# axruff/cuda-flow3d

Hardware: AMD Instinct MI355X
Metric: Mvoxels/s full pyramid solve (higher is better)
Workload: dtype f32; 1 GPU; 512^3 synthetic translated-Gaussian float32 pair (BASELINE config 4), full coarse-to-fine pyramid (40 levels x 40 outer x 5 inner, alpha 7.5, median 5^3, Gaussian sigma 2), frames resident in HBM (value = device-resident rate); parallelism=1 GPU

## Files before the change

cuda-flow3d_amd/__init__.py:

```python
import atexit
import collections
import contextlib
import ctypes as C
import os
import weakref

import numpy as np

_HERE = os.path.dirname(os.path.abspath(__file__))
_LIBDIR = os.environ.get("F3D_LIBDIR") or os.path.join(_HERE, "lib")

DEFAULT_PARAMS = dict(
    warp_levels_count=40, warp_scale_factor=0.95, outer_iterations_count=40, inner_iterations_count=5,
    equation_alpha=7.5, equation_smoothness=0.001, equation_data=0.001, median_radius=5, gaussian_sigma=2.0,
)


class F3dError(RuntimeError):
    pass


class Size4(C.Structure):
    _fields_ = [("width", C.c_size_t), ("height", C.c_size_t), ("depth", C.c_size_t), ("pitch", C.c_size_t)]

# ... 265 lines not shown
        "f3d_flow_principal_compute": [C.c_void_p, C.c_int, C.c_uint, C.POINTER(_fp), C.POINTER(PrincipalStats)],
        "f3d_flow_principal_end": [C.c_void_p],
        "f3d_flow_polar_compute": [C.c_void_p, C.c_int, C.c_uint, C.POINTER(_fp), C.POINTER(PolarStats)],
        "f3d_flow_polar_end": [C.c_void_p],
        "f3d_flow_inverse_compute": [C.c_void_p, C.c_int, C.c_uint, C.c_float, C.POINTER(_fp), C.POINTER(InverseStats)],
        "f3d_flow_inverse_end": [C.c_void_p],
        "f3d_flow_match_compute": [C.c_void_p, C.c_int, C.c_uint, C.c_uint, C.c_float, C.POINTER(_fp), C.POINTER(CorrelationStats)],
        "f3d_flow_match_end": [C.c_void_p],
        "f3d_motion_solve": [C.POINTER(MotionSums), C.c_int, C.POINTER(MotionFit)],
        "f3d_motion_solve_labels": [C.POINTER(MotionSums), _sz, C.c_int, C.c_ulonglong, C.POINTER(C.c_double), C.POINTER(MotionFit),
                                    C.POINTER(C.c_int)],
        "f3d_flow_motion_compute": [C.c_void_p, C.c_int, C.c_int, C.c_float, C.POINTER(_fp), C.POINTER(MotionFit),
                                    C.POINTER(MotionResidual)],
        "f3d_flow_motion_end": [C.c_void_p],
        "f3d_flow_label_motion_compute": [C.c_void_p, C.c_int, C.POINTER(C.c_int), _sz, C.c_int, C.c_ulonglong, C.POINTER(_fp),
                                          C.POINTER(MotionFit), C.POINTER(C.c_int), C.POINTER(C.c_double), C.POINTER(LabelInfo)],
        "f3d_flow_label_motion_end": [C.c_void_p],
        "f3d_flow_validate_compute": [C.c_void_p, C.c_int, C.c_uint, C.c_float, C.c_float, C.c_uint, C.c_uint, C.c_uint, C.c_float,
                                      C.POINTER(_fp), C.POINTER(ValidateStats)],
        "f3d_flow_validate_end": [C.c_void_p],
        "f3d_op_create": [C.POINTER(C.c_void_p), C.c_char_p], "f3d_op_initialize": [C.c_void_p, C.POINTER(Size4)],
        "f3d_op_execute": [C.c_void_p, C.POINTER(C.c_char_p), C.POINTER(C.c_void_p), _sz],
        "f3d_op_execute_batch": [C.c_void_p, C.POINTER(C.c_char_p), C.POINTER(C.c_void_p), C.POINTER(_sz), _sz],
        "f3d_op_set_slab": [C.c_void_p, _slabp], "f3d_op_destroy": [C.c_void_p],
        "f3d_level_geometry": [_sz, _sz, _sz, C.c_float, C.c_int, C.POINTER(Size4), _fp, _fp, _fp],
        "f3d_gaussian_taps": [C.c_float, _fp, _sz, C.POINTER(_sz)],
        "f3d_raw_read_u8": [C.c_char_p, _sz, _sz, _sz, _fp], "f3d_raw_read_f32": [C.c_char_p, _sz, _sz, _sz, _fp],
        "f3d_raw_write_u8": [C.c_char_p, _fp, _sz, _sz, _sz], "f3d_raw_write_f32": [C.c_char_p, _fp, _sz, _sz, _sz],
        "f3d_vtk_write_flow": [C.c_char_p, _fp, _fp, _fp, _sz, _sz, _sz],
        "f3d_synth_pair": [_sz, _sz, _sz, _fp, _fp],
        "f3d_synth_planes": [_sz, _sz, _sz, _sz, _sz, _fp, _fp, _fp],
        "f3d_slabflow_create": [C.POINTER(C.c_void_p), C.c_int, C.POINTER(C.c_int), C.c_int, C.c_int],
        "f3d_slabflow_initialize": [C.c_void_p, _sz, _sz, _sz],
        "f3d_slabflow_compute": [C.c_void_p, _fp, _fp, pp, _fp, _fp, _fp],
        "f3d_slabflow_upload": [C.c_void_p, _fp, _fp],
        "f3d_slabflow_compute_resident": [C.c_void_p, pp, _fp],
        "f3d_slabflow_download": [C.c_void_p, _fp, _fp, _fp],
        "f3d_slabflow_overlapped_iterations": [C.c_void_p, C.POINTER(_sz)],
        "f3d_slabflow_batched_exchanges": [C.c_void_p, C.POINTER(_sz)],
        "f3d_slabflow_gathered_warps": [C.c_void_p, C.POINTER(_sz)],
        "f3d_slabflow_stage_exchanges": [C.c_void_p, C.POINTER(_sz)],
        "f3d_slabflow_set_exchange_per_stage": [C.c_void_p, C.c_int],
        "f3d_slabflow_destroy": [C.c_void_p],
        "f3d_plan_owned": [C.c_int, C.c_int, C.c_int, C.POINTER(C.c_int), C.POINTER(C.c_int)],
        "f3d_plan_exchange": [C.c_int] * 5 + [C.POINTER(C.c_int)] * 5 + [C.c_int],
        "f3d_plan_resample_source": [C.c_int] * 4 + [C.POINTER(C.c_int)] * 2,
        "f3d_volume_wrap": [C.POINTER(C.c_void_p), _fp, _sz, _sz, _sz], "f3d_volume_destroy": [C.c_void_p],
        "f3d_op_solve_p_last": [C.c_void_p, C.POINTER(C.c_int), C.POINTER(C.c_int), C.POINTER(C.c_int), C.POINTER(_sz), C.POINTER(C.c_int)],
        "f3d_op_solve_p_fused_weights": [C.c_void_p, C.POINTER(C.c_int)],
        "f3d_plan_solve_piecemeal": [_sz, _sz, _sz, C.c_int, C.c_int, C.c_int, C.c_int, C.c_int] + [C.POINTER(C.c_int)] * 5,
        "f3d_plan_sweeps": [C.c_int] * 4 + [C.POINTER(C.c_int)] * 2 + [C.c_int],
        "f3d_pair8_plan": [C.c_int] * 7 + [C.POINTER(C.c_longlong)],
        "f3d_pair8_decode": [C.c_int] * 4 + [C.POINTER(C.c_longlong)] + [C.c_int] * 5 + [C.POINTER(C.c_int)] * 2,
        "f3d_pflow_create": [C.POINTER(C.c_void_p)], "f3d_pflow_initialize": [C.c_void_p, _sz, _sz, _sz],
        "f3d_pflow_compute": [C.c_void_p, _fp, _fp, _sz, _sz, _sz, pp, C.c_int, _fp, _fp, _fp, _fp],
        "f3d_pflow_stats": [C.c_void_p, C.POINTER(_sz), C.POINTER(_sz), C.POINTER(_sz)], "f3d_pflow_destroy": [C.c_void_p],
        "f3d_pflow_set_resident": [C.c_void_p, C.c_int], "f3d_pflow_set_full_pipeline": [C.c_void_p, C.c_int], "f3d_pflow_originals_on_device": [C.c_void_p, C.POINTER(C.c_int)],
        "f3d_pflow_operator_seconds": [C.c_void_p, C.POINTER(C.c_double)],
        "f3d_pflow_levels_registered_inside": [C.c_void_p, C.POINTER(_sz)],
        "f3d_pflow_levels_with_constants_on_device": [C.c_void_p, C.POINTER(_sz)],
        "f3d_host_shutdown": [],
    }
    for name, args in sig.items():
        try:
            fn = getattr(L, name)
        except AttributeError:
            if os.environ.get("F3D_LIBDIR"):
                continue
            raise
        fn.argtypes = args
        fn.restype = C.c_int
    L.f3d_flow_default_params.argtypes = [pp]
    L.f3d_flow_default_params.restype = None
    L.f3d_op_name.argtypes = [C.c_void_p]
    L.f3d_op_name.restype = C.c_char_p
    L.f3d_max_warp_level.argtypes = [_sz, _sz, _sz, C.c_float]
    L.f3d_max_warp_level.restype = _sz
    L.f3d_volume_object.argtypes = [C.c_void_p]
    L.f3d_volume_object.restype = C.c_void_p
    L.f3d_volume_data.argtypes = [C.c_void_p]
    L.f3d_volume_data.restype = C.c_void_p
    L.f3d_piecemeal_budget_bytes.argtypes = []
    L.f3d_piecemeal_budget_bytes.restype = _sz
    if hasattr(L, "f3d_host_last_error"):
        L.f3d_host_last_error.argtypes = []
        L.f3d_host_last_error.restype = C.c_char_p
    _host = L
    return L


def shutdown():
    HostVolume.release_all()
    if _host is not None:
        _host.f3d_host_shutdown()
    elif _hip is not None and _hip.f3d_is_initialized():
        _hip.f3d_comm_destroy()
        _hip.f3d_shutdown()


atexit.register(shutdown)


def check(status, what="f3d call"):
    if status != 0:
        msg = hip().f3d_last_error()
        raise F3dError(f"{what} failed: {msg.decode() if msg else 'status %d' % status}")
# ... 688 lines not shown
    @property
    def object(self):
        return host().f3d_volume_object(self._h)

    @property
    def array(self):
        return HostVolume._storage[host().f3d_volume_data(self._h)][0]

    def destroy(self):
        if self._h:
            fin = getattr(self, "_finalizer", None)
            if fin is not None:
                fin.detach()
            HostVolume._release(self._h.value)
            self._h = C.c_void_p()


def plan_solve_piecemeal(budget_bytes, width, height, depth, inner_iterations, outer_iterations, forced_outer_per_pass=0,
                         overlap_mode=0):
    out = [C.c_int() for _ in range(5)]
    check(host().f3d_plan_solve_piecemeal(budget_bytes, width, height, depth, inner_iterations, outer_iterations,
                                          forced_outer_per_pass, overlap_mode, *[C.byref(o) for o in out]))
    return tuple(o.value for o in out)


def plan_sweeps(inner, fused, tri, carry):
    cap = max(1, inner)
    sweeps, weights = (C.c_int * cap)(), (C.c_int * cap)()
    n = host().f3d_plan_sweeps(inner, int(bool(fused)), int(bool(tri)), int(bool(carry)), sweeps, weights, cap)
    if n < 0:
        raise F3dError("f3d_plan_sweeps failed")
    return [(sweeps[i], bool(weights[i])) for i in range(n)]


Pair8Plan = collections.namedtuple("Pair8Plan", "A a b zc_a zc_b wgs cost tiles")


def pair8_plan(width, rows, planes, ty, zc_limit=None, per_round=0, fold=False):
    out = (C.c_longlong * 8)()
    check(host().f3d_pair8_plan(width, rows, planes, ty, planes if zc_limit is None else zc_limit, per_round, int(bool(fold)), out))
    return Pair8Plan(*[int(v) for v in out])


def pair8_decode(width, rows, ty, fold, plan, xcd_remap, z_lo, z_hi):
    cut = (C.c_longlong * 8)(*plan)
    grid = C.c_int()
    args = (width, rows, ty, int(bool(fold)), cut, int(bool(xcd_remap)), z_lo, z_hi)
    check(host().f3d_pair8_decode(*args, 0, 0, None, C.byref(grid)))
    out = np.empty((grid.value, 6), np.int32)
    check(host().f3d_pair8_decode(*args, 0, grid.value, out.ctypes.data_as(C.POINTER(C.c_int)), None))
    return out


class Operation:

    def __init__(self, name):
        self._h = C.c_void_p()
        if host().f3d_op_create(C.byref(self._h), name.encode()) != 0:
            raise F3dError(f"unknown operation {name!r}")
        self.values = {}

    @property
    def name(self):
        return host().f3d_op_name(self._h).decode()

    def initialize(self, containers=None):
        if containers is None:
            return host().f3d_op_initialize(self._h, None) == 0
        s = containers.size4
        return host().f3d_op_initialize(self._h, C.byref(s)) == 0

    def set_slab(self, slab):
        self._slab = slab
        host().f3d_op_set_slab(self._h, C.byref(slab) if slab is not None else None)

    def execute(self, **params):
        store = {}
        volumes = {}
        for k, v in params.items():
            if isinstance(v, HostVolume):
                volumes[k] = v
            elif k in _PTR_KEYS:
                store[k] = _dp(v)
            elif k in _SIZE_T_KEYS:
                store[k] = _sz(v)
            elif k in _FLOAT_KEYS:
                store[k] = C.c_float(v)
            elif k in _SIZE4_KEYS:
                store[k] = Size4(v[0], v[1], v[2], 0) if not isinstance(v, Size4) else v
            elif k == "max_mag":
                store[k] = _sz(v)
            elif k == "stat":
                store[k] = v
            elif k == "flow_update":
                store[k] = C.c_bool(bool(v))
            else:
                raise TypeError(f"unknown parameter key {k!r}")
        n = len(store) + len(volumes)
        keys = (C.c_char_p * n)(*[k.encode() for k in list(store) + list(volumes)])
        ptrs = (C.c_void_p * n)(*([C.cast(C.byref(v), C.c_void_p) for v in store.values()] +
                                  [C.c_void_p(v.object) for v in volumes.values()]))
        check(host().f3d_op_execute(self._h, keys, ptrs, n), "f3d_op_execute")
        self.values = {k: (v.value if hasattr(v, "value") else v) for k, v in store.items()}
        return self.values

    def execute_batch(self, bags):
# ... 463 lines not shown
```

cuda-flow3d_amd/csrc/f3d_pair8_plan.h:

```cpp
#pragma once

#include <algorithm>
#include <cstdlib>

#if !defined(__HIPCC__) && !defined(__host__)
#define __host__
#define __device__
#define F3D_PAIR8_PLAN_OWN_QUALIFIERS
#endif

constexpr int kPair8Lanes = 64;

__host__ __device__ inline int pair8_tiles_per_chunk(int ntx, int nty, bool fold)
{
  return fold ? (ntx - 1) * nty + (nty + 1) / 2 : ntx * nty;
}
inline bool pair8_folds(int width, int rows, int ty)
{
  const char* e = std::getenv("F3D_PAIR8_FOLD");
  if (e && e[0] == '0') return false;
  const int rem = width % kPair8Lanes;
  return rem >= 1 && rem <= kPair8Lanes / 2 && width > kPair8Lanes && rows > ty;
}

struct Pair8Cut {
  int tiles_a, chunks_a, zc_a;
  int tiles_b, chunks_b, zc_b;
};
__host__ __device__ inline int pair8_cut_wgs(const Pair8Cut& c) { return c.tiles_a * c.chunks_a + c.tiles_b * c.chunks_b; }
__host__ __device__ inline int pair8_cut_grid(const Pair8Cut& c, int xcd_remap)
{
  if (!xcd_remap) return pair8_cut_wgs(c);
  return 8 * ((c.tiles_a * c.chunks_a + 7) / 8 + (c.tiles_b * c.chunks_b + 7) / 8);
}

struct Pair8Wg {
  int tile;
  int tx, ty;
  bool folded;
  int z0, z1;
};

__host__ __device__ inline bool pair8_decode(int wg, const Pair8Cut& c, int ntx, int nty, bool fold, int xcd_remap, int m_lo,
                                             int m_hi, int more, Pair8Wg& w)
{
  const int n_a = c.tiles_a * c.chunks_a, n_b = c.tiles_b * c.chunks_b;
  bool in_a;
  int item;
  if (xcd_remap) {
    const int per_a = (n_a + 7) / 8, per_b = (n_b + 7) / 8;
    const int xcd = wg % 8, s = wg / 8;
    in_a = s < per_a;
    item = in_a ? xcd * per_a + s : xcd * per_b + (s - per_a);
  } else {
    in_a = wg < n_a;
    item = in_a ? wg : wg - n_a;
  }
  if (item >= (in_a ? n_a : n_b)) return false;
  const int tiles = in_a ? c.tiles_a : c.tiles_b, zc = in_a ? c.zc_a : c.zc_b;
  const int chunk = item / tiles;
  w.tile = item % tiles + (in_a ? 0 : c.tiles_a);
  w.z0 = m_lo + chunk * zc;
  w.z1 = w.z0 + zc + more < m_hi ? w.z0 + zc + more : m_hi;
  if (fold) {
    const int pair = w.tile / (2 * ntx - 1), k = w.tile % (2 * ntx - 1);
    w.folded = k == ntx - 1;
    w.tx = k < ntx ? k : k - ntx;
    w.ty = k < ntx ? 2 * pair : 2 * pair + 1;
  } else {
    w.folded = false;
    w.tx = w.tile % ntx;
    w.ty = w.tile / ntx;
  }
  return true;
}

struct Pair8Plan {
  int zchunk;
  long cost;
  long wgs = 0;
  Pair8Cut cut = {};
};
inline Pair8Cut pair8_uniform_cut(int tiles, int planes, int zchunk)
{
  return Pair8Cut{0, 0, 0, tiles, (planes + zchunk - 1) / zchunk, zchunk};
}
inline long pair8_per_round(long standard)
{
  const char* e = std::getenv("F3D_PAIR8_ROUND");
  const long v = e ? std::atol(e) : 0;
  return v > 0 ? v : standard;
}
inline Pair8Plan pair8_plan_dims(int width, int rows, int planes, int ty, int zc_limit, long per_round = 256, bool fold = false,
                                 bool two_class = true)
{
  const long tiles = pair8_tiles_per_chunk((width + kPair8Lanes - 1) / kPair8Lanes, (rows + ty - 1) / ty, fold);
  const int max_chunks = planes > 0 ? planes : 1;
  static const int extra = std::getenv("F3D_PAIR8_CHUNK_STEPS") ? std::atoi(std::getenv("F3D_PAIR8_CHUNK_STEPS")) : 7;
  auto rounds = [&](long wgs) { return (wgs + per_round - 1) / per_round; };
  Pair8Plan p = {std::min(planes, zc_limit), -1};
  for (int nzc = 1; nzc <= max_chunks; ++nzc) {
    const int zc = (planes + nzc - 1) / nzc;
    if (zc > zc_limit) continue;
    const long wgs = tiles * ((planes + zc - 1) / zc);
    const long cost = rounds(wgs) * (zc + extra);
    if (p.cost < 0 || cost < p.cost) {
      p.cost = cost;
      p.zchunk = zc;
      p.wgs = wgs;
    }
  }
  if (p.cost < 0) {
    p.cost = static_cast<long>(rounds(tiles)) * (p.zchunk + extra);
    p.wgs = tiles;
  }
  if (p.zchunk < 1) p.zchunk = 1;
  p.cut = pair8_uniform_cut(static_cast<int>(tiles), planes, p.zchunk);
  const char* pe = std::getenv("F3D_PAIR8_PLAN");
  if (!two_class || (pe && pe[0] == '0') || tiles <= per_round || planes < 1 || zc_limit < 1) return p;
  const int a0 = (planes + zc_limit - 1) / zc_limit;
  int zc_a_seen = 0;
  for (int na = a0; na <= a0 + 2 && na <= planes; ++na) {
    const int zc_a = (planes + na - 1) / na;
    if (zc_a > zc_limit || zc_a == zc_a_seen) continue;
    zc_a_seen = zc_a;
    const int a = (planes + zc_a - 1) / zc_a;
    long g = a, r = per_round;
    while (r) { const long t = g % r; g = r; r = t; }
    const long stride = per_round / g;
    for (long A = stride; A < tiles; A += stride) {
      const long cost_a = rounds(A * a) * (zc_a + extra);
      if (cost_a >= p.cost) break;
      int zc_b_seen = 0;
      for (int nb = 1; nb <= planes; ++nb) {
        const int zc_b = (planes + nb - 1) / nb;
        if (zc_b > zc_limit || zc_b == zc_b_seen) continue;
        zc_b_seen = zc_b;
        const int b = (planes + zc_b - 1) / zc_b;
        const long cost = cost_a + rounds((tiles - A) * b) * (zc_b + extra);
        if (cost < p.cost) {
          p.cost = cost;
          p.wgs = A * a + (tiles - A) * b;
          p.cut = Pair8Cut{static_cast<int>(A), a, zc_a, static_cast<int>(tiles - A), b, zc_b};
        }
      }
    }
  }
  return p;
}

#ifdef F3D_PAIR8_PLAN_OWN_QUALIFIERS
#undef __host__
#undef __device__
#undef F3D_PAIR8_PLAN_OWN_QUALIFIERS
#endif
```

cuda-flow3d_amd/csrc/f3d_solve_pair8.h:

```cpp

enum { PAIR_SS = 0, PAIR_SP = 1 };

struct PairArgs {
  const float* in[12];
  float* out[5];
  float hx, hy, hz, alpha;
  float eps_s, eps_d;
  int plain_division;
  int keep_below, keep_above;
  double r4[3], r2[3];
  float d4[3], d2[3];
  float w[3];
  float eps_s2, eps_d2;
  int fdivs_ok, sdivs_ok;
};

inline bool pair_weights_finite(float hx, float hy, float hz, float alpha)
{
  for (float h : {hx, hy, hz}) {
    const float w = alpha / (h * h);
    if (!(w - w == 0.f) || std::signbit(w)) return false;
  }
  return true;
}
// ... 656 lines not shown
    fetch_neighbours(colw_c, Sp);
  };

  __syncthreads();
  PlaneRegs A = {}, B = {}, Cc = {};
  const float* Sm = &ring[0][0];
  const float* S0 = &ring[1][0];
  using Slot0 = std::integral_constant<int, 0>;
  using Slot1 = std::integral_constant<int, 1>;
  using Slot2 = std::integral_constant<int, 2>;
  auto march = [&](auto colw_c) __attribute__((always_inline)) {
    constexpr bool CW = decltype(colw_c)::value;
    if constexpr (CW) {
      halo_raw(A, Sm, side, jc, e_near, false);
      halo_raw(B, S0, side, jc, e_near, true, &cring[0][0]);
    } else {
      row_raw(A, Sm, jr, false);
      row_raw(B, S0, jr, true, &cring[0][0]);
    }
    plane_finish(A);
    plane_finish(B);
    fetch_neighbours(colw_c, S0);
    int q = qs;
    for (; q + 2 <= q_end; q += 3) {
      step(colw_c, Slot2{}, A, B, Cc, q);
      step(colw_c, Slot0{}, B, Cc, A, q + 1);
      step(colw_c, Slot1{}, Cc, A, B, q + 2);
    }
    if (q <= q_end) step(colw_c, Slot2{}, A, B, Cc, q);
    if (q + 1 <= q_end) step(colw_c, Slot0{}, B, Cc, A, q + 1);
  };
  if (colw) march(std::true_type{});
  else march(std::false_type{});
  asm volatile("s_waitcnt vmcnt(0)" ::: "memory");
  };
  if constexpr (FOLDS) {
    if (__builtin_amdgcn_readfirstlane(static_cast<int>(folded))) return tile_body(std::true_type{});
  }
  tile_body(std::false_type{});
}

template <int MODE, int TY, int ABL = 0, bool FD = false, bool YM = false, bool FOLDS = false>
__global__ __launch_bounds__(kLanes*(TY + 4)) void k_pair8(PairArgs a, F3dGeo g, Pair8Cut cut, int ntx, int nty, int xcd_remap)
{
  pair8_body<MODE, TY, ABL, FD, YM, false, FOLDS>(a, g, cut, ntx, nty, xcd_remap);
}
template <int MODE, int TY>
__global__ __launch_bounds__(kLanes*(TY + 2)) __attribute__((amdgpu_waves_per_eu(4))) void k_pair8t(PairArgs a, F3dGeo g, Pair8Cut cut, int ntx,
                                                                                                   int nty, int xcd_remap)
{
  pair8_body<MODE, TY, 0, false, true, true>(a, g, cut, ntx, nty, xcd_remap);
}

inline Pair8Plan pair8_plan(const F3dGeo& g, int ty, long per_round = 256)
{
  return pair8_plan_dims(g.W, g.H, g.z_hi - g.z_lo, ty, max_planes_per_chunk(g), pair8_per_round(per_round), pair8_folds(g.W, g.H, ty));
}

inline int pair8_ymarch_rows(const F3dGeo& g)
{
  const char* e = std::getenv("F3D_PAIR8_YMARCH");
  const int mode = e ? std::atoi(e) : -1;
  if (mode == 0) return 0;
  if (g.z_base != 0 || g.z_lo != 0 || g.z_hi != g.D || g.D > 8 || g.D < 2 || g.H < 2) return 0;
  const unsigned long long bytes = static_cast<unsigned long long>(g.Hc) * static_cast<unsigned long long>(g.pitch) * 4ull *
                                   static_cast<unsigned long long>(g.D + 1);
  if (bytes >= 0xf0000000ull) return 0;
  const char* te = std::getenv("F3D_PAIR8_TIGHT");
  const bool tight = !(te && te[0] == '0');
  const int min_planes = tight ? 4 : 5;
  if (mode != 1 && (g.D < min_planes || g.H < 8 * g.D)) return 0;
  return g.D <= 4 ? 4 : (g.D == 5 ? 5 : 8);
}

template <int MODE, int TY, bool FD = false, bool YM = false, bool TIGHT = false>
void launch_pair8(const PairArgs& args, const F3dGeo& g, int force_zchunk, int xcd_remap)
{
  PairArgs a = args;
  pair_consts(a);
  const int rows = YM ? g.D : g.H;
  const int planes = YM ? g.H : g.z_hi - g.z_lo;
  const int ntx = (g.W + kLanes - 1) / kLanes;
  const int nty = (rows + TY - 1) / TY;
  const int zc_limit = YM ? planes : max_planes_per_chunk(g);
#ifdef F3D_LAB
  static const int abl = std::getenv("F3D_ABLATE8") ? std::atoi(std::getenv("F3D_ABLATE8")) : 0;
#else
  constexpr int abl = 0;
#endif
  const int fold = !YM && abl == 0 && pair8_folds(g.W, rows, TY) ? 1 : 0;
  const int tiles = pair8_tiles_per_chunk(ntx, nty, fold != 0);
  Pair8Cut cut = pair8_plan_dims(g.W, rows, planes, TY, zc_limit, pair8_per_round(TIGHT ? 512 : 256), fold != 0, !YM && abl == 0).cut;
  if (force_zchunk > 0) cut = pair8_uniform_cut(tiles, planes, std::min(force_zchunk, zc_limit));
  const dim3 grid(pair8_cut_grid(cut, xcd_remap), 1, 1), block(kLanes, TY + (TIGHT ? 2 : 4), 1);
  auto go = [&](auto kern) { hipLaunchKernelGGL(kern, grid, block, 0, f3d::stream(), a, g, cut, ntx, nty, xcd_remap); };
  if constexpr (!YM) {
    if (fold) return go(k_pair8<MODE, TY, 0, FD, false, true>);
  }
  if constexpr (YM && TIGHT) return go(k_pair8t<MODE, TY>);
  else if constexpr (YM) return go(k_pair8<MODE, TY, 0, false, true>);
  else if constexpr (FD) return go(k_pair8<MODE, TY, 0, true>);
  else {
#ifdef F3D_LAB
    if constexpr (TY == 12) {
      if (abl == 16) return go(k_pair8<MODE, TY, 16>);
    }
    if constexpr (MODE == PAIR_SS) {
      if (abl == 1) return go(k_pair8<MODE, TY, 1>);
      if (abl == 2) return go(k_pair8<MODE, TY, 2>);
      if (abl == 3) return go(k_pair8<MODE, TY, 3>);
      if (abl == 4) return go(k_pair8<MODE, TY, 4>);
      if (abl == 8) return go(k_pair8<MODE, TY, 8>);
      if (abl == 40) return go(k_pair8<MODE, TY, 40>);
      if constexpr (TY <= 8) {
        if (abl == 64) return go(k_pair8<MODE, TY, 64>);
      }
    }
#endif
    go(k_pair8<MODE, TY, 0>);
  }
}

template <int MODE>
bool launch_pair8_ymarch(const PairArgs& a, const F3dGeo& g, int force_zchunk, int xcd_remap)
{
  const char* e = std::getenv("F3D_PAIR8_TIGHT");
  const bool tight = !(e && e[0] == '0');
  switch (pair8_ymarch_rows(g)) {
    case 4:
      if (tight && g.D == 4) launch_pair8<MODE, 4, false, true, true>(a, g, force_zchunk, xcd_remap);
      else launch_pair8<MODE, 4, false, true>(a, g, force_zchunk, xcd_remap);
      return true;
    case 5:
      if (tight && g.D == 5) launch_pair8<MODE, 5, false, true, true>(a, g, force_zchunk, xcd_remap);
      else launch_pair8<MODE, 5, false, true>(a, g, force_zchunk, xcd_remap);
      return true;
    case 8: launch_pair8<MODE, 8, false, true>(a, g, force_zchunk, xcd_remap); return true;
    default: return false;
  }
}
```

cuda-flow3d_amd/host/host_capi.cpp:

```cpp
#include <cstring>
#include <memory>
#include <new>
#include <string>
#include <vector>

#include "f3d_host.h"
#include "hip_utils.h"
#include "motion_fit.h"
#include "operations.h"
#include "operations_p.h"
#include "optical_flow.h"
#include "optical_flow_p.h"
#include "optical_flow_slab.h"
#include "synth.h"
#include "../csrc/f3d_pair8_plan.h"

struct f3d_flow_s {
  OpticalFlowE driver;
  bool device_ready = false;
  bool trajectory_started = false;
  bool zncc_of_held_flow = false;
};

struct f3d_slabflow_s {
// ... 601 lines not shown
  return 0;
}

int f3d_pflow_destroy(f3d_pflow flow)
{
  delete flow;
  return 0;
}

size_t f3d_piecemeal_budget_bytes(void) { return PiecemealBudgetBytes(); }

int f3d_plan_solve_piecemeal(size_t budget_bytes, size_t width, size_t height, int depth, int inner_iterations, int outer_iterations,
                             int forced_outer_per_pass, int overlap_mode, int* chunk, int* outer_per_pass, int* halo, int* max_planes,
                             int* overlapped)
{
  const SolvePiecemealPlan plan = PlanSolvePiecemeal(budget_bytes, width, height, depth, inner_iterations, outer_iterations,
                                                     forced_outer_per_pass, overlap_mode);
  if (overlapped) *overlapped = plan.overlapped ? 1 : 0;
  if (chunk) *chunk = plan.chunk;
  if (outer_per_pass) *outer_per_pass = plan.outer_per_pass;
  if (halo) *halo = plan.halo;
  if (max_planes) *max_planes = plan.max_planes;
  return 0;
}

int f3d_plan_sweeps(int inner, int fused, int tri, int carry, int* sweeps, int* next_weights, int capacity)
{
  const std::vector<SweepLaunch> cut = CutSweeps(inner, fused != 0, tri != 0, carry != 0);
  if (static_cast<int>(cut.size()) > capacity || (!cut.empty() && (!sweeps || !next_weights))) return -1;
  for (size_t i = 0; i < cut.size(); ++i) {
    sweeps[i] = cut[i].sweeps;
    next_weights[i] = cut[i].next_weights ? 1 : 0;
  }
  return static_cast<int>(cut.size());
}

int f3d_pair8_plan(int width, int rows, int planes, int ty, int zc_limit, int per_round, int fold, long long* plan)
{
  if (!plan || width < 1 || rows < 1 || planes < 1 || ty < 1 || zc_limit < 1) return 1;
  const Pair8Plan p = pair8_plan_dims(width, rows, planes, ty, zc_limit, per_round > 0 ? per_round : pair8_per_round(256), fold != 0);
  const long long v[8] = {p.cut.tiles_a, p.cut.chunks_a, p.cut.chunks_b, p.cut.zc_a, p.cut.zc_b, pair8_cut_wgs(p.cut), p.cost,
                          p.cut.tiles_a + p.cut.tiles_b};
  std::copy(v, v + 8, plan);
  return 0;
}

int f3d_pair8_decode(int width, int rows, int ty, int fold, const long long* plan, int xcd_remap, int z_lo, int z_hi, int first,
                     int count, int* out, int* grid)
{
  if (!plan || width < 1 || rows < 1 || ty < 1 || z_hi <= z_lo || first < 0 || count < 0 || (count && !out)) return 1;
  const int ntx = (width + kPair8Lanes - 1) / kPair8Lanes, nty = (rows + ty - 1) / ty;
  const int tiles = pair8_tiles_per_chunk(ntx, nty, fold != 0);
  const Pair8Cut cut = {static_cast<int>(plan[0]), static_cast<int>(plan[1]), static_cast<int>(plan[3]),
                        tiles - static_cast<int>(plan[0]), static_cast<int>(plan[2]), static_cast<int>(plan[4])};
  if (cut.tiles_a < 0 || cut.tiles_b < 0 || (cut.tiles_a && (cut.chunks_a < 1 || cut.zc_a < 1)) ||
      (cut.tiles_b && (cut.chunks_b < 1 || cut.zc_b < 1)))
    return 1;
  if (grid) *grid = pair8_cut_grid(cut, xcd_remap);
  for (int i = 0; i < count; ++i) {
    Pair8Wg w;
    int* o = out + 6 * static_cast<size_t>(i);
    if (pair8_decode(first + i, cut, ntx, nty, fold != 0, xcd_remap, z_lo, z_hi, 0, w)) {
      o[0] = w.tile; o[1] = w.tx; o[2] = w.ty; o[3] = w.folded ? 1 : 0; o[4] = w.z0; o[5] = w.z1;
    } else {
      std::fill(o, o + 6, -1);
    }
  }
  return 0;
}

size_t f3d_max_warp_level(size_t width, size_t height, size_t depth, float scale_factor)
{
  return OpticalFlowBase::GetMaxWarpLevel(width, height, depth, scale_factor);
}

int f3d_level_geometry(size_t width, size_t height, size_t depth, float scale_factor, int level, f3d_size4* size,
                       float* hx, float* hy, float* hz)
{
  if (!size || !hx || !hy || !hz) return 1;
  DataSize4 original = {width, height, depth, 0};
  PyramidLevel lv = OpticalFlowBase::GetLevel(original, scale_factor, level);
  *size = {lv.size.width, lv.size.height, lv.size.depth, 0};
  *hx = lv.hx;
  *hy = lv.hy;
  *hz = lv.hz;
  return 0;
}

int f3d_gaussian_taps(float sigma, float* taps, size_t capacity, size_t* radius)
{
  if (!taps || !radius) return 1;
  CudaOperationConvolution3D conv;
  conv.ComputeGaussianKernel(sigma, 3, 1.0);
  const size_t n = 2 * conv.KernelRadius() + 1;
  if (n > capacity || n > 51) return 1;
  std::memcpy(taps, conv.Kernel(), n * sizeof(float));
  *radius = conv.KernelRadius();
  return 0;
}

int f3d_raw_read_u8(const char* path, size_t width, size_t height, size_t depth, float* out)
{
  Data3D vol;
  if (!vol.ReadRAWFromFileU8(path, width, height, depth)) return 1;
  std::memcpy(out, vol.DataPtr(), width * height * depth * sizeof(float));
  return 0;
}

int f3d_raw_read_f32(const char* path, size_t width, size_t height, size_t depth, float* out)
{
  Data3D vol;
  if (!vol.ReadRAWFromFileF32(path, width, height, depth)) return 1;
  std::memcpy(out, vol.DataPtr(), width * height * depth * sizeof(float));
  return 0;
}

int f3d_raw_write_u8(const char* path, const float* in, size_t width, size_t height, size_t depth)
{
  Data3D vol(const_cast<float*>(in), width, height, depth);
  return vol.WriteRAWToFileU8(path) ? 0 : 1;
}

int f3d_raw_write_f32(const char* path, const float* in, size_t width, size_t height, size_t depth)
// ... 182 lines not shown
```

include/f3d_host.h:

```cpp
#ifndef F3D_HOST_H_
#define F3D_HOST_H_

#include "f3d.h"

#ifdef __cplusplus
extern "C" {
#endif

typedef struct f3d_flow_params {
  size_t warp_levels_count;
  float  warp_scale_factor;
  size_t outer_iterations_count;
  size_t inner_iterations_count;
  float  equation_alpha;
  float  equation_smoothness;
  float  equation_data;
  size_t median_radius;
  float  gaussian_sigma;
} f3d_flow_params;

typedef struct f3d_flow_s* f3d_flow;
typedef struct f3d_op_s* f3d_op;

void f3d_flow_default_params(f3d_flow_params* p);
// ... 42 lines not shown
                             f3d_inverse_stats* stats);
int f3d_flow_inverse_end(f3d_flow flow);

#define F3D_MATCH_WARPED 1u
#define F3D_MATCH_ZNCC 2u
#define F3D_MATCH_RMSD 4u
int f3d_flow_match_compute(f3d_flow flow, int source, unsigned fields, unsigned radius, float threshold, float* const out[3],
                           f3d_correlation_stats* stats);
int f3d_flow_match_end(f3d_flow flow);

int f3d_motion_solve(const struct f3d_motion_sums* sums, int model, f3d_motion_fit* fit);

int f3d_motion_solve_labels(const struct f3d_motion_sums* sums, size_t n_labels, int model, unsigned long long min_voxels,
                            const double volume_centre[3], f3d_motion_fit* fits, int* status);

int f3d_flow_motion_compute(f3d_flow flow, int source, int model, float min_zncc, float* const out[3], f3d_motion_fit* fit,
                            f3d_motion_residual* residual);
int f3d_flow_motion_end(f3d_flow flow);

int f3d_flow_label_motion_compute(f3d_flow flow, int source, const int* labels, size_t n_labels, int model, unsigned long long min_voxels,
                                  float* const out[3], f3d_motion_fit* fits, int* status, double* rms_after ,
                                  f3d_label_info* info );
int f3d_flow_label_motion_end(f3d_flow flow);

int f3d_flow_validate_compute(f3d_flow flow, int source, unsigned step, float eps, float threshold, unsigned min_neighbours,
                              unsigned mode, unsigned fill_passes, float min_zncc, float* const out[4], f3d_validate_stats* stats);
int f3d_flow_validate_end(f3d_flow flow);
const char* f3d_host_last_error(void);
int f3d_flow_destroy(f3d_flow flow);

int f3d_op_create(f3d_op* op, const char* name);
const char* f3d_op_name(f3d_op op);
int f3d_op_initialize(f3d_op op, const f3d_size4* container_size);
int f3d_op_execute(f3d_op op, const char* const* keys, void* const* value_ptrs, size_t count);
int f3d_op_execute_batch(f3d_op op, const char* const* keys, void* const* value_ptrs, const size_t* counts, size_t bags);
int f3d_op_set_slab(f3d_op op, const f3d_slab* slab);
int f3d_op_destroy(f3d_op op);

typedef struct f3d_volume_s* f3d_volume;
int f3d_volume_wrap(f3d_volume* vol, float* data, size_t width, size_t height, size_t depth);
void* f3d_volume_object(f3d_volume vol);
float* f3d_volume_data(f3d_volume vol);
int f3d_volume_destroy(f3d_volume vol);
int f3d_op_solve_p_last(f3d_op op, int* chunk, int* outer_per_pass, int* halo, size_t* passes, int* overlapped);
int f3d_op_solve_p_fused_weights(f3d_op op, int* fused);
int f3d_plan_solve_piecemeal(size_t budget_bytes, size_t width, size_t height, int depth, int inner_iterations, int outer_iterations,
                             int forced_outer_per_pass, int overlap_mode, int* chunk, int* outer_per_pass, int* halo, int* max_planes,
                             int* overlapped);
size_t f3d_piecemeal_budget_bytes(void);
int f3d_plan_sweeps(int inner, int fused, int tri, int carry, int* sweeps, int* next_weights, int capacity);
int f3d_pair8_plan(int width, int rows, int planes, int ty, int zc_limit, int per_round, int fold, long long* plan);
int f3d_pair8_decode(int width, int rows, int ty, int fold, const long long* plan, int xcd_remap, int z_lo, int z_hi, int first,
                     int count, int* out, int* grid);

typedef struct f3d_pflow_s* f3d_pflow;
int f3d_pflow_create(f3d_pflow* flow);
int f3d_pflow_initialize(f3d_pflow flow, size_t width, size_t height, size_t depth);
int f3d_pflow_compute(f3d_pflow flow, const float* frame_0, const float* frame_1, size_t width, size_t height, size_t depth,
                      const f3d_flow_params* params, int silent, float* u, float* v, float* w, float* device_seconds);
int f3d_pflow_stats(f3d_pflow flow, size_t* solve_passes, size_t* streamed_levels, size_t* resident_levels);
int f3d_pflow_levels_registered_inside(f3d_pflow flow, size_t* levels);
int f3d_pflow_levels_with_constants_on_device(f3d_pflow flow, size_t* levels);
int f3d_pflow_originals_on_device(f3d_pflow flow, int* yes);
int f3d_pflow_set_full_pipeline(f3d_pflow flow, int enabled);
int f3d_pflow_set_resident(f3d_pflow flow, int enabled);
int f3d_pflow_operator_seconds(f3d_pflow flow, double* seconds6);
int f3d_pflow_destroy(f3d_pflow flow);

size_t f3d_max_warp_level(size_t width, size_t height, size_t depth, float scale_factor);
int f3d_level_geometry(size_t width, size_t height, size_t depth, float scale_factor, int level,
                       f3d_size4* size, float* hx, float* hy, float* hz);
int f3d_gaussian_taps(float sigma, float* taps, size_t capacity, size_t* radius);
int f3d_raw_read_u8(const char* path, size_t width, size_t height, size_t depth, float* out);
int f3d_raw_read_f32(const char* path, size_t width, size_t height, size_t depth, float* out);
int f3d_raw_write_u8(const char* path, const float* in, size_t width, size_t height, size_t depth);
int f3d_raw_write_f32(const char* path, const float* in, size_t width, size_t height, size_t depth);
int f3d_vtk_write_flow(const char* path, const float* u, const float* v, const float* w, size_t width, size_t height,
                       size_t depth);
int f3d_synth_pair(size_t width, size_t height, size_t depth, float* frame_0, float* frame_1);
int f3d_synth_planes(size_t width, size_t height, size_t depth, size_t z_lo, size_t z_hi, float* frame_0, float* frame_1,
                     float* frame_0_max);


typedef struct f3d_slabflow_s* f3d_slabflow;

int f3d_slabflow_create(f3d_slabflow* flow, int n_ranks, const int* local_ranks, int n_local, int halo_capacity);
int f3d_slabflow_initialize(f3d_slabflow flow, size_t width, size_t height, size_t depth);
int f3d_slabflow_compute(f3d_slabflow flow, const float* frame_0, const float* frame_1, const f3d_flow_params* params,
                         float* u, float* v, float* w);
int f3d_slabflow_upload(f3d_slabflow flow, const float* frame_0, const float* frame_1);
int f3d_slabflow_compute_resident(f3d_slabflow flow, const f3d_flow_params* params, float* device_seconds);
int f3d_slabflow_download(f3d_slabflow flow, float* u, float* v, float* w);
int f3d_slabflow_overlapped_iterations(f3d_slabflow flow, size_t* count);
int f3d_slabflow_batched_exchanges(f3d_slabflow flow, size_t* count);
int f3d_slabflow_gathered_warps(f3d_slabflow flow, size_t* count);
int f3d_slabflow_stage_exchanges(f3d_slabflow flow, size_t* count);
int f3d_slabflow_set_exchange_per_stage(f3d_slabflow flow, int per_stage);
int f3d_slabflow_destroy(f3d_slabflow flow);

int f3d_plan_owned(int depth, int rank, int n_ranks, int* lo, int* hi);
int f3d_plan_exchange(int depth, int rank, int n_ranks, int need_lo, int need_hi, int* peer, int* send_lo, int* send_hi,
                      int* recv_lo, int* recv_hi, int capacity);
int f3d_plan_resample_source(int in_depth, int out_depth, int out_lo, int out_hi, int* lo, int* hi);

#ifdef __cplusplus
}
// ... 3 lines not shown
```

Baseline: 76.29 Mvoxels/s.

## Add three-class pair8 work partition planner and cache launch plans per tile height

Extends the pair8 solver's workgroup partition from two tile classes to three, each with its own z-chunk size. A memoised search picks the split that minimises estimated rounds times chunk cost, aiming to reduce tail imbalance across CUs. The search is expensive, so launch plans are now cached per geometry and tile-height slot instead of recomputed every launch. Cut fields are made wave-uniform with readfirstlane, and the decode adds a third branch to the kernel's index arithmetic.

New measurement: 77.25 Mvoxels/s, median of 6. 1.3% higher.

```diff
diff --git a/cuda-flow3d_amd/__init__.py b/cuda-flow3d_amd/__init__.py
--- a/cuda-flow3d_amd/__init__.py
+++ b/cuda-flow3d_amd/__init__.py
@@ -341,6 +341,8 @@
         "f3d_plan_sweeps": [C.c_int] * 4 + [C.POINTER(C.c_int)] * 2 + [C.c_int],
         "f3d_pair8_plan": [C.c_int] * 7 + [C.POINTER(C.c_longlong)],
         "f3d_pair8_decode": [C.c_int] * 4 + [C.POINTER(C.c_longlong)] + [C.c_int] * 5 + [C.POINTER(C.c_int)] * 2,
+        "f3d_pair8_plan_wide": [C.c_int] * 7 + [C.POINTER(C.c_longlong)],
+        "f3d_pair8_decode_wide": [C.c_int] * 4 + [C.POINTER(C.c_longlong)] + [C.c_int] * 5 + [C.POINTER(C.c_int)] * 2,
         "f3d_pflow_create": [C.POINTER(C.c_void_p)], "f3d_pflow_initialize": [C.c_void_p, _sz, _sz, _sz],
         "f3d_pflow_compute": [C.c_void_p, _fp, _fp, _sz, _sz, _sz, pp, C.c_int, _fp, _fp, _fp, _fp],
         "f3d_pflow_stats": [C.c_void_p, C.POINTER(_sz), C.POINTER(_sz), C.POINTER(_sz)], "f3d_pflow_destroy": [C.c_void_p],
@@ -1135,6 +1137,27 @@
     return out
 
 
+Pair8WidePlan = collections.namedtuple("Pair8WidePlan", "classes cost wgs tiles")
+
+
+def pair8_plan_wide(width, rows, planes, ty, zc_limit=None, per_round=0, fold=False):
+    out = (C.c_longlong * 12)()
+    check(host().f3d_pair8_plan_wide(width, rows, planes, ty, planes if zc_limit is None else zc_limit, per_round, int(bool(fold)), out))
+    v = [int(x) for x in out]
+    return Pair8WidePlan(tuple(tuple(v[i:i + 3]) for i in (0, 3, 6) if v[i]), v[10], v[9], v[11])
+
+
+def pair8_decode_wide(width, rows, ty, fold, plan, xcd_remap, z_lo, z_hi):
+    classes = [c for c in plan.classes] + [(0, 0, 0)] * (3 - len(plan.classes))
+    cut = (C.c_longlong * 9)(*[x for c in classes for x in c])
+    grid = C.c_int()
+    args = (width, rows, ty, int(bool(fold)), cut, int(bool(xcd_remap)), z_lo, z_hi)
+    check(host().f3d_pair8_decode_wide(*args, 0, 0, None, C.byref(grid)))
+    out = np.empty((grid.value, 6), np.int32)
+    check(host().f3d_pair8_decode_wide(*args, 0, grid.value, out.ctypes.data_as(C.POINTER(C.c_int)), None))
+    return out
+
+
 class Operation:
 
     def __init__(self, name):
diff --git a/cuda-flow3d_amd/csrc/f3d_pair8_plan.h b/cuda-flow3d_amd/csrc/f3d_pair8_plan.h
--- a/cuda-flow3d_amd/csrc/f3d_pair8_plan.h
+++ b/cuda-flow3d_amd/csrc/f3d_pair8_plan.h
@@ -2,6 +2,7 @@
 
 #include <algorithm>
 #include <cstdlib>
+#include <vector>
 
 #if !defined(__HIPCC__) && !defined(__host__)
 #define __host__
@@ -11,6 +12,12 @@
 
 constexpr int kPair8Lanes = 64;
 
+#if defined(__HIP_DEVICE_COMPILE__)
+#define PAIR8_UNIFORM(x) __builtin_amdgcn_readfirstlane(x)
+#else
+#define PAIR8_UNIFORM(x) (x)
+#endif
+
 __host__ __device__ inline int pair8_tiles_per_chunk(int ntx, int nty, bool fold)
 {
   return fold ? (ntx - 1) * nty + (nty + 1) / 2 : ntx * nty;
@@ -26,12 +33,16 @@
 struct Pair8Cut {
   int tiles_a, chunks_a, zc_a;
   int tiles_b, chunks_b, zc_b;
+  int tiles_c, chunks_c, zc_c;
 };
-__host__ __device__ inline int pair8_cut_wgs(const Pair8Cut& c) { return c.tiles_a * c.chunks_a + c.tiles_b * c.chunks_b; }
+__host__ __device__ inline int pair8_cut_wgs(const Pair8Cut& c)
+{
+  return c.tiles_a * c.chunks_a + c.tiles_b * c.chunks_b + c.tiles_c * c.chunks_c;
+}
 __host__ __device__ inline int pair8_cut_grid(const Pair8Cut& c, int xcd_remap)
 {
   if (!xcd_remap) return pair8_cut_wgs(c);
-  return 8 * ((c.tiles_a * c.chunks_a + 7) / 8 + (c.tiles_b * c.chunks_b + 7) / 8);
+  return 8 * ((c.tiles_a * c.chunks_a + 7) / 8 + (c.tiles_b * c.chunks_b + 7) / 8 + (c.tiles_c * c.chunks_c + 7) / 8);
 }
 
 struct Pair8Wg {
@@ -44,22 +55,25 @@
 __host__ __device__ inline bool pair8_decode(int wg, const Pair8Cut& c, int ntx, int nty, bool fold, int xcd_remap, int m_lo,
                                              int m_hi, int more, Pair8Wg& w)
 {
-  const int n_a = c.tiles_a * c.chunks_a, n_b = c.tiles_b * c.chunks_b;
-  bool in_a;
+  const int tiles_a = PAIR8_UNIFORM(c.tiles_a), tiles_b = PAIR8_UNIFORM(c.tiles_b), tiles_c = PAIR8_UNIFORM(c.tiles_c);
+  const int zc_a = PAIR8_UNIFORM(c.zc_a), zc_b = PAIR8_UNIFORM(c.zc_b), zc_c = PAIR8_UNIFORM(c.zc_c);
+  const int n_a = tiles_a * PAIR8_UNIFORM(c.chunks_a), n_b = tiles_b * PAIR8_UNIFORM(c.chunks_b), n_c = tiles_c * PAIR8_UNIFORM(c.chunks_c);
+  int cls;
   int item;
   if (xcd_remap) {
-    const int per_a = (n_a + 7) / 8, per_b = (n_b + 7) / 8;
+    const int per_a = (n_a + 7) / 8, per_b = (n_b + 7) / 8, per_c = (n_c + 7) / 8;
     const int xcd = wg % 8, s = wg / 8;
-    in_a = s < per_a;
-    item = in_a ? xcd * per_a + s : xcd * per_b + (s - per_a);
+    cls = s < per_a ? 0 : (s < per_a + per_b ? 1 : 2);
+    item = cls == 0 ? xcd * per_a + s : (cls == 1 ? xcd * per_b + (s - per_a) : xcd * per_c + (s - per_a - per_b));
   } else {
-    in_a = wg < n_a;
-    item = in_a ? wg : wg - n_a;
-  }
-  if (item >= (in_a ? n_a : n_b)) return false;
-  const int tiles = in_a ? c.tiles_a : c.tiles_b, zc = in_a ? c.zc_a : c.zc_b;
+    cls = wg < n_a ? 0 : (wg < n_a + n_b ? 1 : 2);
+    item = cls == 0 ? wg : (cls == 1 ? wg - n_a : wg - n_a - n_b);
+  }
+  if (item >= (cls == 0 ? n_a : (cls == 1 ? n_b : n_c))) return false;
+  const int tiles = cls == 0 ? tiles_a : (cls == 1 ? tiles_b : tiles_c);
+  const int zc = cls == 0 ? zc_a : (cls == 1 ? zc_b : zc_c);
   const int chunk = item / tiles;
-  w.tile = item % tiles + (in_a ? 0 : c.tiles_a);
+  w.tile = item % tiles + (cls == 0 ? 0 : (cls == 1 ? tiles_a : tiles_a + tiles_b));
   w.z0 = m_lo + chunk * zc;
   w.z1 = w.z0 + zc + more < m_hi ? w.z0 + zc + more : m_hi;
   if (fold) {
@@ -83,7 +97,7 @@
 };
 inline Pair8Cut pair8_uniform_cut(int tiles, int planes, int zchunk)
 {
-  return Pair8Cut{0, 0, 0, tiles, (planes + zchunk - 1) / zchunk, zchunk};
+  return Pair8Cut{0, 0, 0, tiles, (planes + zchunk - 1) / zchunk, zchunk, 0, 0, 0};
 }
 inline long pair8_per_round(long standard)
 {
@@ -91,12 +105,16 @@
   const long v = e ? std::atol(e) : 0;
   return v > 0 ? v : standard;
 }
-inline Pair8Plan pair8_plan_dims(int width, int rows, int planes, int ty, int zc_limit, long per_round = 256, bool fold = false,
-                                 bool two_class = true)
+inline int pair8_chunk_steps()
+{
+  static const int extra = std::getenv("F3D_PAIR8_CHUNK_STEPS") ? std::atoi(std::getenv("F3D_PAIR8_CHUNK_STEPS")) : 7;
+  return extra;
+}
+inline Pair8Plan pair8_plan_two(int width, int rows, int planes, int ty, int zc_limit, long per_round, bool fold, bool two_class)
 {
   const long tiles = pair8_tiles_per_chunk((width + kPair8Lanes - 1) / kPair8Lanes, (rows + ty - 1) / ty, fold);
   const int max_chunks = planes > 0 ? planes : 1;
-  static const int extra = std::getenv("F3D_PAIR8_CHUNK_STEPS") ? std::atoi(std::getenv("F3D_PAIR8_CHUNK_STEPS")) : 7;
+  const int extra = pair8_chunk_steps();
   auto rounds = [&](long wgs) { return (wgs + per_round - 1) / per_round; };
   Pair8Plan p = {std::min(planes, zc_limit), -1};
   for (int nzc = 1; nzc <= max_chunks; ++nzc) {
@@ -116,8 +134,7 @@
   }
   if (p.zchunk < 1) p.zchunk = 1;
   p.cut = pair8_uniform_cut(static_cast<int>(tiles), planes, p.zchunk);
-  const char* pe = std::getenv("F3D_PAIR8_PLAN");
-  if (!two_class || (pe && pe[0] == '0') || tiles <= per_round || planes < 1 || zc_limit < 1) return p;
+  if (!two_class || tiles <= per_round || planes < 1 || zc_limit < 1) return p;
   const int a0 = (planes + zc_limit - 1) / zc_limit;
   int zc_a_seen = 0;
   for (int na = a0; na <= a0 + 2 && na <= planes; ++na) {
@@ -141,12 +158,105 @@
         if (cost < p.cost) {
           p.cost = cost;
           p.wgs = A * a + (tiles - A) * b;
-          p.cut = Pair8Cut{static_cast<int>(A), a, zc_a, static_cast<int>(tiles - A), b, zc_b};
+          p.cut = Pair8Cut{static_cast<int>(A), a, zc_a, static_cast<int>(tiles - A), b, zc_b, 0, 0, 0};
         }
       }
     }
   }
   return p;
+}
+
+inline Pair8Plan pair8_plan_dims(int width, int rows, int planes, int ty, int zc_limit, long per_round = 256, bool fold = false,
+                                 bool two_class = true)
+{
+  const char* pe = std::getenv("F3D_PAIR8_PLAN");
+  return pair8_plan_two(width, rows, planes, ty, zc_limit, per_round, fold, two_class && !(pe && pe[0] == '0'));
+}
+
+inline Pair8Plan pair8_plan_wide(int width, int rows, int planes, int ty, int zc_limit, long per_round = 256, bool fold = false)
+{
+  Pair8Plan best = pair8_plan_two(width, rows, planes, ty, zc_limit, per_round, fold, true);
+  const int tiles = pair8_tiles_per_chunk((width + kPair8Lanes - 1) / kPair8Lanes, (rows + ty - 1) / ty, fold);
+  if (tiles < 2 || planes < 1 || zc_limit < 1 || per_round < 1) return best;
+  const int extra = pair8_chunk_steps();
+  auto rounds = [&](long wgs) { return (wgs + per_round - 1) / per_round; };
+
+  struct Class { int tiles, chunks, zc; };
+  struct Lead { int chunks, zc; long stride; };
+  Lead leads[16];
+  int n_leads = 0;
+  const int a0 = (planes + zc_limit - 1) / zc_limit;
+  for (int na = a0, seen = 0; na < a0 + 16 && na <= planes; ++na) {
+    const int zc = (planes + na - 1) / na;
+    if (zc > zc_limit || zc == seen) continue;
+    seen = zc;
+    const int a = (planes + zc - 1) / zc;
+    long g = a, r = per_round;
+    while (r) { const long t = g % r; g = r; r = t; }
+    leads[n_leads++] = Lead{a, zc, per_round / g};
+  }
+  struct Tail { long cost = -1; Class lead = {0, 0, 0}, last = {0, 0, 0}; };
+  std::vector<Tail> one(tiles + 1), two(tiles + 1);
+  auto uniform = [&](int n) -> const Tail& {
+    Tail& t = one[n];
+    if (t.cost >= 0) return t;
+    for (int nzc = 1, seen = 0; nzc <= planes; ++nzc) {
+      const int zc = (planes + nzc - 1) / nzc;
+      if (zc > zc_limit || zc == seen) continue;
+      seen = zc;
+      const int b = (planes + zc - 1) / zc;
+      const long cost = rounds(static_cast<long>(n) * b) * (zc + extra);
+      if (t.cost < 0 || cost < t.cost) {
+        t.cost = cost;
+        t.last = Class{n, b, zc};
+      }
+    }
+    return t;
+  };
+  auto lead_and_uniform = [&](int n) -> const Tail& {
+    Tail& t = two[n];
+    if (t.cost >= 0) return t;
+    t = uniform(n);
+    for (int i = 0; i < n_leads; ++i) {
+      for (long A = leads[i].stride; A < n; A += leads[i].stride) {
+        const long cost_a = rounds(A * leads[i].chunks) * (leads[i].zc + extra);
+        if (cost_a >= t.cost) break;
+        const Tail& rest = uniform(n - static_cast<int>(A));
+        if (cost_a + rest.cost < t.cost) {
+          t.cost = cost_a + rest.cost;
+          t.lead = Class{static_cast<int>(A), leads[i].chunks, leads[i].zc};
+          t.last = rest.last;
+        }
+      }
+    }
+    return t;
+  };
+  auto take = [&](long cost, const Class& a, const Class& b, const Class& c) {
+    best.cost = cost;
+    best.cut = Pair8Cut{a.tiles, a.chunks, a.zc, b.tiles, b.chunks, b.zc, c.tiles, c.chunks, c.zc};
+    best.wgs = pair8_cut_wgs(best.cut);
+  };
+  {
+    const Tail& t = lead_and_uniform(tiles);
+    if (t.cost < best.cost) take(t.cost, t.lead, t.last, Class{0, 0, 0});
+  }
+  for (int i = 0; i < n_leads; ++i) {
+    for (long A = leads[i].stride; A < tiles; A += leads[i].stride) {
+      const long cost_a = rounds(A * leads[i].chunks) * (leads[i].zc + extra);
+      if (cost_a >= best.cost) break;
+      const Tail& rest = lead_and_uniform(tiles - static_cast<int>(A));
+      if (rest.lead.tiles && cost_a + rest.cost < best.cost)
+        take(cost_a + rest.cost, Class{static_cast<int>(A), leads[i].chunks, leads[i].zc}, rest.lead, rest.last);
+    }
+  }
+  return best;
+}
+
+inline Pair8Plan pair8_plan_launch(int width, int rows, int planes, int ty, int zc_limit, long per_round = 256, bool fold = false)
+{
+  const char* pe = std::getenv("F3D_PAIR8_PLAN");
+  if (pe && (pe[0] == '0' || pe[0] == '1')) return pair8_plan_two(width, rows, planes, ty, zc_limit, per_round, fold, pe[0] == '1');
+  return pair8_plan_wide(width, rows, planes, ty, zc_limit, per_round, fold);
 }
 
 #ifdef F3D_PAIR8_PLAN_OWN_QUALIFIERS
diff --git a/cuda-flow3d_amd/csrc/f3d_solve_pair8.h b/cuda-flow3d_amd/csrc/f3d_solve_pair8.h
--- a/cuda-flow3d_amd/csrc/f3d_solve_pair8.h
+++ b/cuda-flow3d_amd/csrc/f3d_solve_pair8.h
@@ -732,9 +732,33 @@
   pair8_body<MODE, TY, 0, false, true, true>(a, g, cut, ntx, nty, xcd_remap);
 }
 
+inline Pair8Plan pair8_plan_launch_kept(int width, int rows, int planes, int ty, int zc_limit, long per_round, bool fold)
+{
+  struct Key {
+    int width, rows, planes, ty, zc_limit, fold, plan;
+    long per_round;
+    bool operator==(const Key& o) const
+    {
+      return width == o.width && rows == o.rows && planes == o.planes && ty == o.ty && zc_limit == o.zc_limit && fold == o.fold &&
+             plan == o.plan && per_round == o.per_round;
+    }
+  };
+  thread_local Key keys[3] = {};
+  thread_local Pair8Plan plans[3] = {};
+  const char* pe = std::getenv("F3D_PAIR8_PLAN");
+  const Key key = {width, rows, planes, ty, zc_limit, fold ? 1 : 0, pe ? pe[0] : 0, per_round};
+  const int slot = ty <= 4 ? 0 : (ty <= 8 ? 1 : 2);
+  if (!(keys[slot] == key)) {
+    plans[slot] = pair8_plan_launch(width, rows, planes, ty, zc_limit, per_round, fold);
+    keys[slot] = key;
+  }
+  return plans[slot];
+}
+
 inline Pair8Plan pair8_plan(const F3dGeo& g, int ty, long per_round = 256)
 {
-  return pair8_plan_dims(g.W, g.H, g.z_hi - g.z_lo, ty, max_planes_per_chunk(g), pair8_per_round(per_round), pair8_folds(g.W, g.H, ty));
+  return pair8_plan_launch_kept(g.W, g.H, g.z_hi - g.z_lo, ty, max_planes_per_chunk(g), pair8_per_round(per_round),
+                                pair8_folds(g.W, g.H, ty));
 }
 
 inline int pair8_ymarch_rows(const F3dGeo& g)
@@ -770,7 +794,9 @@
 #endif
   const int fold = !YM && abl == 0 && pair8_folds(g.W, rows, TY) ? 1 : 0;
   const int tiles = pair8_tiles_per_chunk(ntx, nty, fold != 0);
-  Pair8Cut cut = pair8_plan_dims(g.W, rows, planes, TY, zc_limit, pair8_per_round(TIGHT ? 512 : 256), fold != 0, !YM && abl == 0).cut;
+  const long per_round = pair8_per_round(TIGHT ? 512 : 256);
+  Pair8Cut cut = !YM && abl == 0 ? pair8_plan_launch_kept(g.W, rows, planes, TY, zc_limit, per_round, fold != 0).cut
+                                 : pair8_plan_two(g.W, rows, planes, TY, zc_limit, per_round, fold != 0, false).cut;
   if (force_zchunk > 0) cut = pair8_uniform_cut(tiles, planes, std::min(force_zchunk, zc_limit));
   const dim3 grid(pair8_cut_grid(cut, xcd_remap), 1, 1), block(kLanes, TY + (TIGHT ? 2 : 4), 1);
   auto go = [&](auto kern) { hipLaunchKernelGGL(kern, grid, block, 0, f3d::stream(), a, g, cut, ntx, nty, xcd_remap); };
diff --git a/cuda-flow3d_amd/host/host_capi.cpp b/cuda-flow3d_amd/host/host_capi.cpp
--- a/cuda-flow3d_amd/host/host_capi.cpp
+++ b/cuda-flow3d_amd/host/host_capi.cpp
@@ -677,7 +677,7 @@
   const int ntx = (width + kPair8Lanes - 1) / kPair8Lanes, nty = (rows + ty - 1) / ty;
   const int tiles = pair8_tiles_per_chunk(ntx, nty, fold != 0);
   const Pair8Cut cut = {static_cast<int>(plan[0]), static_cast<int>(plan[1]), static_cast<int>(plan[3]),
-                        tiles - static_cast<int>(plan[0]), static_cast<int>(plan[2]), static_cast<int>(plan[4])};
+                        tiles - static_cast<int>(plan[0]), static_cast<int>(plan[2]), static_cast<int>(plan[4]), 0, 0, 0};
   if (cut.tiles_a < 0 || cut.tiles_b < 0 || (cut.tiles_a && (cut.chunks_a < 1 || cut.zc_a < 1)) ||
       (cut.tiles_b && (cut.chunks_b < 1 || cut.zc_b < 1)))
     return 1;
@@ -694,6 +694,41 @@
   return 0;
 }
 
+int f3d_pair8_plan_wide(int width, int rows, int planes, int ty, int zc_limit, int per_round, int fold, long long* plan)
+{
+  if (!plan || width < 1 || rows < 1 || planes < 1 || ty < 1 || zc_limit < 1) return 1;
+  const Pair8Plan p = pair8_plan_launch(width, rows, planes, ty, zc_limit, per_round > 0 ? per_round : pair8_per_round(256), fold != 0);
+  const Pair8Cut& c = p.cut;
+  const long long v[12] = {c.tiles_a, c.chunks_a, c.zc_a, c.tiles_b, c.chunks_b, c.zc_b, c.tiles_c, c.chunks_c, c.zc_c,
+                           pair8_cut_wgs(c), p.cost, c.tiles_a + c.tiles_b + c.tiles_c};
+  std::copy(v, v + 12, plan);
+  return 0;
+}
+
+int f3d_pair8_decode_wide(int width, int rows, int ty, int fold, const long long* plan, int xcd_remap, int z_lo, int z_hi, int first,
+                          int count, int* out, int* grid)
+{
+  if (!plan || width < 1 || rows < 1 || ty < 1 || z_hi <= z_lo || first < 0 || count < 0 || (count && !out)) return 1;
+  const int ntx = (width + kPair8Lanes - 1) / kPair8Lanes, nty = (rows + ty - 1) / ty;
+  int v[9];
+  for (int i = 0; i < 9; ++i) v[i] = static_cast<int>(plan[i]);
+  const Pair8Cut cut = {v[0], v[1], v[2], v[3], v[4], v[5], v[6], v[7], v[8]};
+  for (int i = 0; i < 9; i += 3)
+    if (v[i] < 0 || (v[i] && (v[i + 1] < 1 || v[i + 2] < 1))) return 1;
+  if (cut.tiles_a + cut.tiles_b + cut.tiles_c != pair8_tiles_per_chunk(ntx, nty, fold != 0)) return 1;
+  if (grid) *grid = pair8_cut_grid(cut, xcd_remap);
+  for (int i = 0; i < count; ++i) {
+    Pair8Wg w;
+    int* o = out + 6 * static_cast<size_t>(i);
+    if (pair8_decode(first + i, cut, ntx, nty, fold != 0, xcd_remap, z_lo, z_hi, 0, w)) {
+      o[0] = w.tile; o[1] = w.tx; o[2] = w.ty; o[3] = w.folded ? 1 : 0; o[4] = w.z0; o[5] = w.z1;
+    } else {
+      std::fill(o, o + 6, -1);
+    }
+  }
+  return 0;
+}
+
 size_t f3d_max_warp_level(size_t width, size_t height, size_t depth, float scale_factor)
 {
   return OpticalFlowBase::GetMaxWarpLevel(width, height, depth, scale_factor);
diff --git a/include/f3d_host.h b/include/f3d_host.h
--- a/include/f3d_host.h
+++ b/include/f3d_host.h
@@ -118,6 +118,9 @@
 int f3d_pair8_plan(int width, int rows, int planes, int ty, int zc_limit, int per_round, int fold, long long* plan);
 int f3d_pair8_decode(int width, int rows, int ty, int fold, const long long* plan, int xcd_remap, int z_lo, int z_hi, int first,
                      int count, int* out, int* grid);
+int f3d_pair8_plan_wide(int width, int rows, int planes, int ty, int zc_limit, int per_round, int fold, long long* plan);
+int f3d_pair8_decode_wide(int width, int rows, int ty, int fold, const long long* plan, int xcd_remap, int z_lo, int z_hi, int first,
+                          int count, int* out, int* grid);
 
 typedef struct f3d_pflow_s* f3d_pflow;
 int f3d_pflow_create(f3d_pflow* flow);
```
